# vlaxose/jstsp19

Hardware: AMD Instinct MI355X
Metric: channel-estimates/sec (batched MC) at Nt=Nr=64,K=64; NMSE vs ref (higher is better)
Workload: dtype c32 (storage and results fp32 complex; big contractions as split-f16 MFMA with fp32 accumulation, fp32-equivalent); 1 GPU; proposed_algorithm approximate Imax=100, Nt=Nr=64 Nrf=8 K=64 L=8 (N=64 M=4096 Gr=64 G2=512); Imax=100, outputs=S,Y,convergence_error, pilots=per-trial (B per trial), parallelism=trials sharded, dp1

## Files before the change

### jstsp19_amd/csrc/common.h

```cpp
#pragma once
#include <hip/hip_runtime.h>
#include <cstdint>
#include <cstdio>
#include <cstdarg>
#include <string>
#include <vector>
#include <map>
#include "../../include/jstsp.h"

namespace jstsp {

void set_error(const char *fmt, ...);

#define JSTSP_HIP(call)                                                                  \
    do {                                                                                 \
        hipError_t e_ = (call);                                                          \
        if (e_ != hipSuccess) {                                                          \
            jstsp::set_error("%s failed: %s (%s:%d)", #call, hipGetErrorString(e_),      \
                             __FILE__, __LINE__);                                        \
            return (int)e_;                                                              \
        }                                                                                \
    } while (0)

#define JSTSP_TRY(expr)                                                                  \
// ... 146 lines not shown
    bool profiling = false;
    std::map<std::string, jstsp::ProfileSlot> prof;
    std::vector<hipEvent_t> event_pool;
    int num_cus = 256;
    void *pinned = nullptr;
    size_t pinned_cap = 0, pinned_off = 0;
    hipEvent_t pinned_done = nullptr;
    bool pinned_pending = false;
    uint32_t *diag = nullptr;
    unsigned *lz_mismatch = nullptr;
    void *hpin = nullptr;
    size_t hpin_cap = 0;
    hipEvent_t hpin_done = nullptr;
    bool hpin_pending = false;
    int dict_block_hint = 0;
    int last_dict_block = 0;
    int fused_fallbacks = 0;
    float2 *unit = nullptr;
    double2 *unit64 = nullptr;
    jstsp_ctx *helper = nullptr;
    hipStream_t side[2] = {nullptr, nullptr};
    hipStream_t cu_stream[4] = {nullptr, nullptr, nullptr, nullptr};
    int cu_state = 0;
    hipStream_t bj_stream[3] = {nullptr, nullptr, nullptr};
    hipEvent_t bj_ev[6] = {nullptr, nullptr, nullptr, nullptr, nullptr, nullptr};
    hipEvent_t ev[10] = {nullptr, nullptr, nullptr, nullptr, nullptr, nullptr, nullptr, nullptr, nullptr, nullptr};
};

namespace jstsp {

struct GemmDesc {
    const float2 *A; long long sAt, sAi, sAk; int conjA;
    const float2 *B; long long sBt, sBk, sBj; int conjB;
    const float2 *B2;
    float2 *C; long long sCt; int ldc;
    const float2 *D; long long sDt; int ldd;
    float alpha, beta;
    int m, n, k, batch;
    int splitk; long long sCsplit;
    int epi;
    const TrialParams *prm;
    float2 *e_rw0, *e_w1, *e_w2, *e_w3;
    const float2 *e_r0, *e_r1, *e_r2, *e_r3;
    const float *e_f0;
    int epi_store_c;
    uint32_t *amax_x, *amax_v1, *amax_z;
// ... 3 lines not shown
    int herm_upper;
    int sa_mode;
    const float *sa_lr, *sa_lt;
    float sa_rho, sa_thr;
};
__device__ __forceinline__ float sadmm_den(float lr, float lt, float rho) { return fmaf(lr, lt, -rho); }
__device__ __forceinline__ float sadmm_dual1(float z, float r, float s, float rho) { return fmaf(rho, r - s, z); }
__device__ __forceinline__ float sadmm_soft1(float r, float z, float ir, float thr)
{
    const float v = fmaf(ir, z, r);
    const float m = fmaxf(fabsf(v) - thr, 0.f);
    return (v > 0.f) ? m : ((v < 0.f) ? -m : 0.f);
}
__device__ __forceinline__ float sadmm_rhs1(float z, float s, float a, float rho) { return fmaf(-rho, s, z) + a; }
enum { EPI_NONE = 0, EPI_UPDATE_C = 1, EPI_UPDATE_X = 2, EPI_SADMM = 3 };
enum { GEMM_MISC = 0, GEMM_CORRELATE = 1, GEMM_SYNTH = 2, GEMM_GRAM = 3 };
int launch_cgemm(jstsp_ctx *ctx, const GemmDesc &d, int tag = GEMM_MISC);

struct HPack {
    uint4 *data = nullptr;
    uint32_t *bmax = nullptr;
    int KS = 0, JT = 0, count = 0;
    long long st = 0;
};
struct HGemmDesc {
    const float2 *A; long long sAt, sAk;
    const uint32_t *amax;
    const uint4 *Bp; long long sPt;
    const uint32_t *bmax; int sbmax;
    int KS, JT;
    float2 *C; long long sCt; int ldc;
    int m, n, k, batch;
    int epi;
    const TrialParams *prm;
    const float2 *e_r0;
    float2 *e_rw0;
    uint32_t *amax_v2;
    const uint4 *Ap; long long sApt; int aKS;
    int herm_upper;
    int map_tb, map_tt;
};
int hermitian_fill_lower(jstsp_ctx *ctx, float2 *G, long long sGt, int n, int count);
int launch_hgram(jstsp_ctx *ctx, const float2 *Z, long long sZt, int rows, int cols, int count, int nsplit,
                 const uint32_t *amax, float2 *Gpart, const float2 *Z2 = nullptr,
                 const TrialParams *zprm = nullptr,
                 bool norm_only = false);
int launch_hgram3(jstsp_ctx *ctx, const float2 *X, const float2 *V1, long long sZt, int rows, int cols, int count, int nsplit,
                  const uint32_t *xmax, const uint32_t *vmax, const uint32_t *zmax, const TrialParams *prm, float2 *Gz,
                  float2 *Gx, float2 *Gv);
size_t hgemm_pack_bytes(int Kd, int J, int count);
bool hgemm_pair_shape(int m, int n, int batch);
int hgemm_absmax(jstsp_ctx *ctx, const float2 *X, long long n, long long sXt, int count, uint32_t *amax);
int hgemm_pack(jstsp_ctx *ctx, HPack &p, Arena &ar, const float2 *B, long long sBt, long long sBk, long long sBj,
               int conj, int Kd, int J, int count, long long n_contig, const uint32_t *bmax_known = nullptr);
int hgemm_repack(jstsp_ctx *ctx, const HPack &p, const float2 *B, long long sBt, long long sBk, long long sBj, int conj,
                 int Kd, int J, const uint32_t *bmax);
int launch_hgemm(jstsp_ctx *ctx, const HGemmDesc &d, const char *prof_name = nullptr);
bool use_hgemm(long long m, long long n, long long k);

enum { EIG_SVT_Q = 0, EIG_LMAX = 1, EIG_VECS = 2 };
int launch_eig(jstsp_ctx *ctx, int mode, int n, int batch, const float2 *Gpart, long long sGt,
               int nsplit, long long sGs, const TrialParams *prm, const float *tau,
               float2 *Q, float *lam_out, float2 *Vg);
bool eig_needs_global_v(int n);
int launch_eig_large(jstsp_ctx *ctx, int mode, int n, int batch, const float2 *Gpart, long long sGt, int nsplit,
                     long long sGs, const TrialParams *prm, const float *tau, float2 *Q, float *lam_out);
int launch_eig_fast(jstsp_ctx *ctx, int mode, int n, int batch, const float2 *Gpart, long long sGt, int nsplit,
                    long long sGs, const TrialParams *prm, const float *tau, float2 *Q, float *lam_out,
                    float2 *Uwarm, int warm);
int launch_eig128(jstsp_ctx *ctx, int n, int batch, const float2 *Gpart, long long sGt, int nsplit, long long sGs,
                  const TrialParams *prm, const float *tau, float2 *Q, float2 *Uwarm = nullptr, int warm = 0,
                  int max_sweeps = 16, float stop_level = 0.f);
int eig_fast_ne(int n);
struct LanczosWarm {
    float2 *x = nullptr;
    int *state = nullptr;
    unsigned *mismatch = nullptr;
// ... 32 lines not shown
```

### jstsp19_amd/csrc/hgemm.hip

```cpp
#include "solver_common.h"
#include <type_traits>

namespace jstsp {

typedef _Float16 half8 __attribute__((ext_vector_type(8)));
typedef float f32x16 __attribute__((ext_vector_type(16)));
typedef unsigned int u32x4 __attribute__((ext_vector_type(4)));

namespace {

constexpr int HBK = 32;
constexpr int FLUSH = 8;
constexpr float LO_SCALE = 1.f, LO_INV = 1.f;

__device__ __host__ inline int scale_exp(uint32_t amax_bits)
{
    const int be = (int)((amax_bits >> 23) & 0xff);
    if (be == 0 || be == 255) return 0;
    return 13 - (be - 127);
}

__device__ __forceinline__ void split2(float x, _Float16 &h, _Float16 &l)
{
    h = (_Float16)x;
// ... 6 lines not shown
    const float *p = X + (long long)t * sXt;
    float m = 0.f;
    const bool vec = ((sXt & 3) == 0) && ((n2 & 3) == 0) && (((uintptr_t)X & 15) == 0);
    if (vec) {
        const float4 *p4 = reinterpret_cast<const float4 *>(p);
        for (long long i = (long long)blockIdx.x * 256 + threadIdx.x; i < n2 / 4; i += (long long)gridDim.x * 256) {
            const float4 v = p4[i];
            m = fmaxf(fmaxf(m, fmaxf(fabsf(v.x), fabsf(v.y))), fmaxf(fabsf(v.z), fabsf(v.w)));
        }
    } else {
        for (long long i = (long long)blockIdx.x * 256 + threadIdx.x; i < n2; i += (long long)gridDim.x * 256)
            m = fmaxf(m, fabsf(p[i]));
    }
    for (int o = 32; o > 0; o >>= 1) m = fmaxf(m, __shfl_xor(m, o));
    __shared__ float sm[4];
    if ((threadIdx.x & 63) == 0) sm[threadIdx.x >> 6] = m;
    __syncthreads();
    if (threadIdx.x == 0)
        atomicMax(&amax[t], __float_as_uint(fmaxf(fmaxf(sm[0], sm[1]), fmaxf(sm[2], sm[3]))));
}

__global__ __launch_bounds__(256) void pack_b_kernel(const float2 *B, long long sBt, long long sBk, long long sBj,
                                                     int conj, int Kd, int J, int KS, int JT, const uint32_t *bmax,
                                                     uint4 *out)
{
    const int t = blockIdx.y;
    const long long idx = (long long)blockIdx.x * 256 + threadIdx.x;
    if (idx >= (long long)JT * KS * 64) return;
    const int lane = (int)(idx & 63);
    const long long blk = idx >> 6;
    const int ks = (int)(blk % KS), jt = (int)(blk / KS);
    const int j = jt * 32 + (lane & 31), k0 = ks * 16 + 8 * (lane >> 5);
    const float s = ldexpf(1.f, scale_exp(bmax[t]));
    const float sg = conj ? -s : s;
    half8 rh, rl, ih, il;
#pragma unroll
    for (int v = 0; v < 8; ++v) {
        float2 x = make_float2(0.f, 0.f);
        if (j < J && k0 + v < Kd) x = B[(long long)t * sBt + (long long)(k0 + v) * sBk + (long long)j * sBj];
        _Float16 h, l;
        split2(x.x * s, h, l); rh[v] = h; rl[v] = l;
        split2(x.y * sg, h, l); ih[v] = h; il[v] = l;
    }
    uint4 *o = out + (((long long)t * JT + jt) * KS + ks) * 256 + lane;
    o[0] = *reinterpret_cast<uint4 *>(&rh);
    o[64] = *reinterpret_cast<uint4 *>(&rl);
    o[128] = *reinterpret_cast<uint4 *>(&ih);
    o[192] = *reinterpret_cast<uint4 *>(&il);
}

__device__ __forceinline__ half8 as_half8(uint4 u) { return *reinterpret_cast<half8 *>(&u); }
__device__ __forceinline__ half8 neg_half8(uint4 u)
{
    u.x ^= 0x80008000u; u.y ^= 0x80008000u; u.z ^= 0x80008000u; u.w ^= 0x80008000u;
    return *reinterpret_cast<half8 *>(&u);
}

__device__ __forceinline__ bool block_to_trial_tile(const HGemmDesc &d, int tiles, int &t, int &tile)
{
    const int bid = blockIdx.x;
    const int xcd = bid & 7, slot = bid >> 3;
    if (d.map_tb == 0) {
        t = (slot / tiles) * 8 + xcd;
        tile = slot % tiles;
        return t < d.batch;
    }
    const int per = d.map_tb * d.map_tt;
    const int nbt = (d.batch + d.map_tb - 1) / d.map_tb;
    const int blk = (slot / per) * 8 + xcd, w = slot % per;
    t = (blk % nbt) * d.map_tb + w % d.map_tb;
    tile = (blk / nbt) * d.map_tt + w / d.map_tb;
    return t < d.batch && tile < tiles;
}

template <int EPI, bool APACK, int WJ, bool EVEN = false>
__global__ __launch_bounds__(128 * WJ, WJ == 2 ? 2 : 2) void hgemm_kernel(HGemmDesc d, int tiles_i, int tiles_j)
{
    constexpr int STG = 1024 + 512 * WJ;
    constexpr int NA = (WJ == 2) ? 8 : 4;
    __shared__ uint4 smem[2 * STG];

    const int tiles = tiles_i * tiles_j;
    int t, rem;
    if (!block_to_trial_tile(d, tiles, t, rem)) return;
    const int ti = rem % tiles_i, tj = rem / tiles_i;
    const int i0 = ti * 64, j0 = tj * 32 * WJ;
    if (d.herm_upper && i0 >= j0 + 32 * WJ) return;

    const int tid = threadIdx.x, lane = tid & 63, wave = tid >> 6;
    const int wi = wave & 1, wj = wave >> 1;

    const int ea = scale_exp(d.amax[t]);
    const int eb = scale_exp(d.bmax[(long long)t * d.sbmax]);
    const float sa = ldexpf(1.f, ea);

    const int ai = tid & 63, akg = tid >> 6;
    const bool arow = (i0 + ai) < d.m;
    const float2 *abase = APACK ? nullptr : d.A + (long long)t * d.sAt;
    const float2 *pa = APACK ? nullptr : abase + (arow ? (i0 + ai) : 0) + (long long)(NA * akg) * d.sAk;
    const int a_slot = (WJ == 2) ? ((((ai >> 5) * 2 + (akg >> 1)) * 4) * 64) + (akg & 1) * 32 + (ai & 31)
                                 : ((((ai >> 5) * 2 + (akg >> 2)) * 4) * 64) + ((akg >> 1) & 1) * 32 + (ai & 31);
    const uint4 *pb = d.Bp + (long long)t * d.sPt + ((long long)(tj * WJ) * d.KS) * 256 + lane;
    const int nst = d.KS / 2;
    const int kfull = d.k / HBK;

    struct StgF { float2 a[NA]; uint4 b0, b1, b2, b3; };
    struct StgP { u32x4 a0, a1, a2, a3; uint4 b0, b1, b2, b3; };
    using Stg = typename std::conditional<APACK, StgP, StgF>::type;
    const uint4 *pbw = pb + ((long long)(wave >> 1) * d.KS + (wave & 1)) * 256;
    const uint4 *paw = APACK ? d.Ap + (long long)t * d.sApt + lane +
                                   ((long long)(ti * 2 + (wave >> 1)) * d.KS + (wave & 1)) * 256
                             : nullptr;
    const float sa_m = arow ? sa : 0.f;
    auto load = [&](int s_in, Stg &R) {
        const int s = EVEN ? (s_in < nst ? s_in : 0) : s_in;
        const uint4 *g = pbw + (long long)(2 * s) * 256;
        const u32x4 *gn = reinterpret_cast<const u32x4 *>(g);
        const u32x4 x0 = __builtin_nontemporal_load(gn), x1 = __builtin_nontemporal_load(gn + 64),
                    x2 = __builtin_nontemporal_load(gn + 128), x3 = __builtin_nontemporal_load(gn + 192);
        R.b0 = make_uint4(x0.x, x0.y, x0.z, x0.w); R.b1 = make_uint4(x1.x, x1.y, x1.z, x1.w);
        R.b2 = make_uint4(x2.x, x2.y, x2.z, x2.w); R.b3 = make_uint4(x3.x, x3.y, x3.z, x3.w);
        if constexpr (APACK) {
            const u32x4 *ga = reinterpret_cast<const u32x4 *>(paw + (long long)(2 * s) * 256);
            R.a0 = ga[0]; R.a1 = ga[64]; R.a2 = ga[128]; R.a3 = ga[192];
        } else {
            if (EVEN || s < kfull) {
#pragma unroll
                for (int v = 0; v < NA; ++v) R.a[v] = pa[(long long)(s * HBK + v) * d.sAk];
            } else {
                const int kbase = s * HBK + NA * akg;
#pragma unroll
                for (int v = 0; v < NA; ++v) {
                    const bool ok = kbase + v < d.k;
                    const float2 *p = ok ? pa + (long long)(s * HBK + v) * d.sAk : abase;
                    const float2 x = *p;
                    R.a[v] = ok ? x : make_float2(0.f, 0.f);
                }
            }
        }
    };
    auto store = [&](const Stg &R, uint4 *buf) {
        uint4 *o = buf + 1024 + wave * 256 + lane;
        o[0] = R.b0; o[64] = R.b1; o[128] = R.b2; o[192] = R.b3;
        if constexpr (APACK) {
            u32x4 *q = reinterpret_cast<u32x4 *>(buf + wave * 256 + lane);
            q[0] = R.a0; q[64] = R.a1; q[128] = R.a2; q[192] = R.a3;
        } else {
            half8 rh = {0}, rl = {0}, ih = {0}, il = {0};
#pragma unroll
            for (int v = 0; v < NA; ++v) {
                _Float16 h, l;
                split2(R.a[v].x * sa_m, h, l); rh[v] = h; rl[v] = l;
                split2(R.a[v].y * sa_m, h, l); ih[v] = h; il[v] = l;
            }
            if constexpr (WJ == 2) {
                uint4 *q = buf + a_slot;
                q[0] = *reinterpret_cast<uint4 *>(&rh);
                q[64] = *reinterpret_cast<uint4 *>(&rl);
                q[128] = *reinterpret_cast<uint4 *>(&ih);
                q[192] = *reinterpret_cast<uint4 *>(&il);
            } else {
                uint2 *q = reinterpret_cast<uint2 *>(buf + a_slot) + (akg & 1);
                q[0] = *reinterpret_cast<uint2 *>(&rh);
                q[2 * 64] = *reinterpret_cast<uint2 *>(&rl);
                q[2 * 128] = *reinterpret_cast<uint2 *>(&ih);
                q[2 * 192] = *reinterpret_cast<uint2 *>(&il);
            }
        }
    };

    f32x16 re_h = {0}, re_l = {0}, im_h = {0}, im_l = {0};
    f32x16 Lre = {0}, Lim = {0};
    auto fold = [&]() {
#pragma unroll
        for (int r = 0; r < 16; ++r) {
            Lre[r] += re_h[r] + re_l[r] * LO_INV;
            Lim[r] += im_h[r] + im_l[r] * LO_INV;
            re_h[r] = 0.f; re_l[r] = 0.f; im_h[r] = 0.f; im_l[r] = 0.f;
        }
    };
    auto compute = [&](const uint4 *buf) {
#pragma unroll
        for (int ks = 0; ks < 2; ++ks) {
            const uint4 *fa = buf + ((wi * 2 + ks) * 4) * 64 + lane;
            const uint4 *fb = buf + 1024 + ((wj * 2 + ks) * 4) * 64 + lane;
            const uint4 uar_h = fa[0], uar_l = fa[64], uai_h = fa[128], uai_l = fa[192];
            const half8 br_h = as_half8(fb[0]), br_l = as_half8(fb[64]), bi_h = as_half8(fb[128]), bi_l = as_half8(fb[192]);
            const half8 ar_h = as_half8(uar_h), ar_l = as_half8(uar_l), ai_h = as_half8(uai_h), ai_l = as_half8(uai_l);
            const half8 nai_h = neg_half8(uai_h), nai_l = neg_half8(uai_l);
            re_h = __builtin_amdgcn_mfma_f32_32x32x16_f16(br_h, ar_h, re_h, 0, 0, 0);
            re_l = __builtin_amdgcn_mfma_f32_32x32x16_f16(br_l, ar_h, re_l, 0, 0, 0);
            im_h = __builtin_amdgcn_mfma_f32_32x32x16_f16(bi_h, ar_h, im_h, 0, 0, 0);
            im_l = __builtin_amdgcn_mfma_f32_32x32x16_f16(bi_l, ar_h, im_l, 0, 0, 0);
            re_h = __builtin_amdgcn_mfma_f32_32x32x16_f16(bi_h, nai_h, re_h, 0, 0, 0);
            re_l = __builtin_amdgcn_mfma_f32_32x32x16_f16(br_h, ar_l, re_l, 0, 0, 0);
            im_h = __builtin_amdgcn_mfma_f32_32x32x16_f16(br_h, ai_h, im_h, 0, 0, 0);
            im_l = __builtin_amdgcn_mfma_f32_32x32x16_f16(bi_h, ar_l, im_l, 0, 0, 0);
            re_l = __builtin_amdgcn_mfma_f32_32x32x16_f16(bi_l, nai_h, re_l, 0, 0, 0);
            im_l = __builtin_amdgcn_mfma_f32_32x32x16_f16(br_l, ai_h, im_l, 0, 0, 0);
            re_l = __builtin_amdgcn_mfma_f32_32x32x16_f16(bi_h, nai_l, re_l, 0, 0, 0);
            im_l = __builtin_amdgcn_mfma_f32_32x32x16_f16(br_h, ai_l, im_l, 0, 0, 0);
        }
    };
    auto stage = [&](int s, const uint4 *cur, uint4 *nxt, Stg &Rnear, Stg &Rfar) {
        if (EVEN || s + 2 < nst) load(s + 2, Rfar);
        compute(cur);
        asm volatile("" ::: "memory");
        __builtin_amdgcn_sched_barrier(0);
        if (EVEN || s + 1 < nst) store(Rnear, nxt);
        if (((s + 1) % FLUSH) == 0) fold();
        __syncthreads();
    };

    Stg R0, R1;
    uint4 *buf0 = smem, *buf1 = smem + STG;
    load(0, R0);
    if (EVEN || nst > 1) load(1, R1);
    store(R0, buf0);
    __syncthreads();

    for (int s = 0; s < nst; s += 2) {
        stage(s, buf0, buf1, R1, R0);
        if (EVEN || s + 1 < nst) stage(s + 1, buf1, buf0, R0, R1);
    }
    fold();

    const float alpha = ldexpf(1.f, -(ea + eb));
    const int gi = i0 + wi * 32 + (lane & 31);
    float2 *Cp = d.C + (long long)t * d.sCt;
    float vmax = 0.f;
    if (gi < d.m) {
#pragma unroll
        for (int r = 0; r < 16; ++r) {
            const int gj = j0 + wj * 32 + (r & 3) + 8 * (r >> 2) + 4 * (lane >> 5);
            if (gj >= d.n) continue;
            const float2 o = make_float2(Lre[r] * alpha, Lim[r] * alpha);
            const long long ix = (long long)t * d.sCt + gi + (long long)gj * d.ldc;
            if (EPI == EPI_UPDATE_C) {
                const TrialParams prm = d.prm[t];
                const float2 x = d.e_r0[ix];
                float2 v2 = d.e_rw0[ix];
                v2.x = admm_v2(prm, v2.x, x.x, o.x);
                v2.y = admm_v2(prm, v2.y, x.y, o.y);
                d.e_rw0[ix] = v2;
                vmax = fmaxf(vmax, fmaxf(fabsf(v2.x), fabsf(v2.y)));
            }
            Cp[gi + (long long)gj * d.ldc] = o;
// ... 786 lines not shown
    JSTSP_HIP(hipGetLastError());
    return 0;
}

int hgemm_pack(jstsp_ctx *ctx, HPack &p, Arena &ar, const float2 *B, long long sBt, long long sBk, long long sBj,
               int conj, int Kd, int J, int count, long long n_contig, const uint32_t *bmax_known)
{
    p.KS = 4 * ((Kd + 63) / 64);
    p.JT = 4 * ((J + 127) / 128);
    p.count = count;
    p.st = (long long)p.JT * p.KS * 256;
    p.data = ar.get<uint4>((size_t)count * p.st);
    p.bmax = ar.get<uint32_t>(count);
    JSTSP_REQUIRE(p.data && p.bmax, JSTSP_E_NOMEM, "workspace exhausted (packed dictionary)");
    if (bmax_known) JSTSP_HIP(hipMemcpyAsync(p.bmax, bmax_known, (size_t)count * sizeof(uint32_t), hipMemcpyDeviceToDevice, ctx->stream));
    else JSTSP_TRY(hgemm_absmax(ctx, B, n_contig, sBt, count, p.bmax));
    const long long slots = (long long)p.JT * p.KS * 64;
    pack_b_kernel<<<dim3((unsigned)((slots + 255) / 256), count), 256, 0, ctx->stream>>>(B, sBt, sBk, sBj, conj, Kd, J,
                                                                                         p.KS, p.JT, p.bmax, p.data);
    JSTSP_HIP(hipGetLastError());
    return 0;
}

int hgemm_repack(jstsp_ctx *ctx, const HPack &p, const float2 *B, long long sBt, long long sBk, long long sBj, int conj,
                 int Kd, int J, const uint32_t *bmax)
{
    const long long slots = (long long)p.JT * p.KS * 64;
    pack_b_kernel<<<dim3((unsigned)((slots + 255) / 256), p.count), 256, 0, ctx->stream>>>(B, sBt, sBk, sBj, conj, Kd, J,
                                                                                           p.KS, p.JT, bmax, p.data);
    JSTSP_HIP(hipGetLastError());
    return 0;
}

int launch_hgram(jstsp_ctx *ctx, const float2 *Z, long long sZt, int rows, int cols, int count, int nsplit,
                 const uint32_t *amax, float2 *Gpart, const float2 *Z2, const TrialParams *zprm, bool norm_only)
{
    JSTSP_REQUIRE(rows > 0 && rows <= 64 && cols > 0 && count > 0 && nsplit > 0, JSTSP_E_SHAPE, "hgram: bad shape");
    const long long grid = (long long)count * nsplit;
    JSTSP_REQUIRE(grid < (1ll << 31), JSTSP_E_UNSUPPORTED, "hgram grid too large");
    prof_begin(ctx, "gram");
    JSTSP_REQUIRE(!Z2 || zprm, JSTSP_E_NULL, "hgram: Z2 without per-problem scalars");
    if (norm_only && !Z2 && cols >= GRAM_HONLY_MIN_COLS) {
        if (cols % (nsplit * 2 * HBK) == 0)
            hgram_kernel<true, true><<<(unsigned)grid, 256, 0, ctx->stream>>>(Z, sZt, rows, cols, nsplit, amax, Gpart, count, Z2, zprm);
        else
            hgram_kernel<false, true><<<(unsigned)grid, 256, 0, ctx->stream>>>(Z, sZt, rows, cols, nsplit, amax, Gpart, count, Z2, zprm);
// ... 63 lines not shown
        d.map_tt = conc / d.map_tb < 1 ? 1 : conc / d.map_tb;
        if (d.map_tt > tiles) d.map_tt = (int)tiles;
        const long long nb = (long long)((d.batch + d.map_tb - 1) / d.map_tb) * ((tiles + d.map_tt - 1) / d.map_tt);
        return ((nb + 7) / 8) * 8 * d.map_tb * d.map_tt;
    }
    return (long long)((d.batch + 7) / 8) * 8 * tiles;
}

bool hgemm_pair_shape(int m, int n, int batch)
{
    return m == 64 && batch >= 2 && (long long)((batch + 1) / 2) * ((n + 127) / 128) >= 256;
}

int launch_hgemm(jstsp_ctx *ctx, const HGemmDesc &d_in, const char *prof_name)
{
    HGemmDesc d = d_in;
    JSTSP_REQUIRE(d.m > 0 && d.n > 0 && d.k > 0 && d.batch > 0, JSTSP_E_SHAPE, "hgemm: bad shape");
    JSTSP_REQUIRE(d.KS >= 2 * ((d.k + 31) / 32) && d.JT >= 2 * ((d.n + 63) / 64), JSTSP_E_ARG,
                  "hgemm: packed operand smaller than the product");
    const bool wide = !d.Ap && d.epi == EPI_NONE && d.n >= 128 && d.JT * 32 >= ((d.n + 127) / 128) * 128;
    const int tiles_i = (d.m + 63) / 64, tiles_j = wide ? (d.n + 127) / 128 : (d.n + 63) / 64;
    const bool wide_even = wide && (d.k % 32) == 0 && ((d.KS / 2) % 2) == 0 && d.KS == 2 * (d.k / 32);
    JSTSP_REQUIRE((long long)((d.batch + 7) / 8) * 8 * tiles_i * tiles_j < (1ll << 30), JSTSP_E_UNSUPPORTED, "hgemm grid too large");
    if (d.Ap && d.aKS == d.KS && d.sPt == 0 && d.sbmax == 0 && !d.herm_upper && (d.KS % 4) == 0 &&
        hgemm_pair_shape(d.m, d.n, d.batch) && d.JT * 32 >= ((d.n + 127) / 128) * 128) {
        const int npairs = (d.batch + 1) / 2, tj3 = (d.n + 127) / 128;
        d.map_tb = npairs < 4 ? npairs : 4;
        d.map_tt = 32 / d.map_tb < tj3 ? 32 / d.map_tb : tj3;
        const long long nb = (long long)((npairs + d.map_tb - 1) / d.map_tb) * ((tj3 + d.map_tt - 1) / d.map_tt);
        const long long grid3 = ((nb + 7) / 8) * 8 * d.map_tb * d.map_tt;
        JSTSP_REQUIRE(grid3 < (1ll << 31), JSTSP_E_UNSUPPORTED, "hgemm grid too large");
        if (prof_name) prof_begin(ctx, prof_name);
        constexpr int PAIR_LDS = 3 * 2048 * (int)sizeof(uint4);
        auto go = [&](auto kern, int lds) -> int {
            JSTSP_HIP(hipFuncSetAttribute(reinterpret_cast<const void *>(kern), hipFuncAttributeMaxDynamicSharedMemorySize, lds));
            hipLaunchKernelGGL(kern, dim3((unsigned)grid3), dim3(256), lds, ctx->stream, d, tj3, npairs);
            return 0;
        };
        if (d.epi == EPI_UPDATE_C) JSTSP_TRY(go(hgemm_pair_kernel<EPI_UPDATE_C, false>, PAIR_LDS));
        else if (d.k > 1024) JSTSP_TRY(go(hgemm_pair_kernel<EPI_NONE, true>, PAIR_LDS + 65536));
        else JSTSP_TRY(go(hgemm_pair_kernel<EPI_NONE, false>, PAIR_LDS));
        if (prof_name) prof_end(ctx, prof_name);
        JSTSP_HIP(hipGetLastError());
        return 0;
    }
    const int v2_mask = 1;
    const bool pack_ok = d.JT * 32 >= ((d.n + 127) / 128) * 128;
    if (d.m <= 64 && pack_ok && d.Ap && (v2_mask & 1) && d.aKS == d.KS && (d.KS % 4) == 0) {
        const int tj2 = (d.n + 127) / 128;
        const long long grid2 = hgemm_grid(d, tj2, 64);
        if (prof_name) prof_begin(ctx, prof_name);
        if (d.epi == EPI_UPDATE_C)
            hgemm2_kernel<EPI_UPDATE_C, true, 4, 2><<<(unsigned)grid2, 256, 0, ctx->stream>>>(d, tj2);
        else
            hgemm2_kernel<EPI_NONE, true, 4, 2><<<(unsigned)grid2, 256, 0, ctx->stream>>>(d, tj2);
        if (prof_name) prof_end(ctx, prof_name);
        JSTSP_HIP(hipGetLastError());
        return 0;
    }
    if (d.m <= 64 && pack_ok && !d.Ap && (v2_mask & 2) && (d.KS % 4) == 0 && d.epi == EPI_NONE && d.k <= 1024) {
        const int tj2 = (d.n + 127) / 128;
        const long long grid2 = hgemm_grid(d, tj2, 64);
        if (prof_name) prof_begin(ctx, prof_name);
        hgemm2_kernel<EPI_NONE, false, 4, 2><<<(unsigned)grid2, 256, 0, ctx->stream>>>(d, tj2);
        if (prof_name) prof_end(ctx, prof_name);
        JSTSP_HIP(hipGetLastError());
        return 0;
    }
    const long long grid = hgemm_grid(d, (long long)tiles_i * tiles_j, wide ? 32 : 64);
    if (prof_name) prof_begin(ctx, prof_name);
    if (wide_even) {
        hgemm_kernel<EPI_NONE, false, 4, true><<<(unsigned)grid, 512, 0, ctx->stream>>>(d, tiles_i, tiles_j);
    } else if (wide) {
        hgemm_kernel<EPI_NONE, false, 4><<<(unsigned)grid, 512, 0, ctx->stream>>>(d, tiles_i, tiles_j);
    } else if (d.Ap) {
        JSTSP_REQUIRE(d.aKS == d.KS, JSTSP_E_ARG, "hgemm: packed a and b operands disagree on the k padding");
        if (d.epi == EPI_UPDATE_C)
            hgemm_kernel<EPI_UPDATE_C, true, 2><<<(unsigned)grid, 256, 0, ctx->stream>>>(d, tiles_i, tiles_j);
        else
            hgemm_kernel<EPI_NONE, true, 2><<<(unsigned)grid, 256, 0, ctx->stream>>>(d, tiles_i, tiles_j);
    } else if (d.epi == EPI_UPDATE_C)
        hgemm_kernel<EPI_UPDATE_C, false, 2><<<(unsigned)grid, 256, 0, ctx->stream>>>(d, tiles_i, tiles_j);
    else
        hgemm_kernel<EPI_NONE, false, 2><<<(unsigned)grid, 256, 0, ctx->stream>>>(d, tiles_i, tiles_j);
    if (prof_name) prof_end(ctx, prof_name);
    JSTSP_HIP(hipGetLastError());
    return 0;
}

}
```

### jstsp19_amd/csrc/proposed.hip

```cpp
#include "solver_common.h"
#include <cstdio>
#include <cmath>
#include <cstdlib>
#include <algorithm>

namespace jstsp {

struct ProposedWS {
    float2 *X, *V1, *V2, *C, *Xs, *Y, *ZK, *Zb, *Zb2;
    float *invD;
    float2 *V, *RV, *Res, *RRes, *S, *P1;
    float2 *Tc, *W;
    float2 *GA, *GB;
    TrialParams *prm;
    int32_t *rank;
    double *ce;
    float *lam;
    GramWS gz, gn;
    bool h2 = false;
    HPack Bc, Bs;
    uint32_t *kmax = nullptr, *wmax = nullptr;
    uint32_t *nmax = nullptr, *zmax = nullptr;
    bool h2g = false;
    HPack GBp;
    HPack Wp;
    HPack Kp;
    uint32_t *pmax = nullptr;
};

static int gram3_nsplit(int N, int M, int G2, bool want_ce)
{
    const int chunk = 1024;
    if (!(want_ce && N <= 64 && N <= M && use_hgemm(N, G2, M))) return 0;
    return std::max(1, std::min(32, (M + chunk - 1) / chunk));
}

static size_t proposed_bytes(int N, int M, int Gr, int G2, int batch, int nA, int nB, bool angles,
                             bool want_ce, int Imax)
{
    const size_t nm = (size_t)N * M, g = (size_t)Gr * G2, ng = (size_t)N * G2;
    size_t b = 0;
    b += rnd256(3 * batch * nm * sizeof(float2)) + 6 * rnd256(batch * nm * sizeof(float2));
    b += rnd256(batch * nm * sizeof(float));
    b += 6 * rnd256(batch * g * sizeof(float2));
    b += 2 * rnd256(batch * ng * sizeof(float2));
    b += rnd256((size_t)nA * Gr * Gr * sizeof(float2)) + rnd256((size_t)nB * G2 * G2 * sizeof(float2));
    b += rnd256(batch * sizeof(TrialParams));
    if (angles) b += rnd256(batch * g * sizeof(int32_t));
    b += rnd256((size_t)batch * 3 * Imax * sizeof(double));
    b += rnd256(3 * (size_t)batch * sizeof(float));
    const int ns3 = gram3_nsplit(N, M, G2, want_ce);
    b += GramWS::bytes(N, M, batch, true, ns3);
    if (want_ce) b += GramWS::bytes(N, M, 3 * batch, false, ns3);
    if (use_hgemm(N, G2, M))
        b += hgemm_pack_bytes(M, G2, nB) + hgemm_pack_bytes(G2, M, nB) + 2 * rnd256(8 * batch * sizeof(uint32_t)) +
             hgemm_pack_bytes(G2, N, batch);
    if (use_hgemm(N, G2, M) && nB == 1 && hgemm_pair_shape(N, G2, batch))
        b += rnd256((size_t)batch * 2 * (4 * ((M + 63) / 64)) * 256 * sizeof(uint4));
    if (use_hgemm(Gr, G2, G2)) b += hgemm_pack_bytes(G2, G2, nB) + rnd256(2 * batch * sizeof(uint32_t));
    return b;
}

static int proposed_alloc(Arena &a, ProposedWS &w, int N, int M, int Gr, int G2, int batch, int nA, int nB,
                          bool angles, bool want_ce, int Imax)
{
    const size_t nm = (size_t)N * M, g = (size_t)Gr * G2, ng = (size_t)N * G2;
    w.X = a.get<float2>(3 * batch * nm);
    w.V1 = w.X ? w.X + batch * nm : nullptr;
    w.V2 = w.X ? w.X + 2 * batch * nm : nullptr;
    w.C = a.get<float2>(batch * nm); w.Xs = a.get<float2>(batch * nm); w.Y = a.get<float2>(batch * nm);
    w.ZK = a.get<float2>(batch * nm);
    w.Zb = a.get<float2>(batch * nm);
    w.Zb2 = a.get<float2>(batch * nm);
    w.invD = a.get<float>(batch * nm);
    w.V = a.get<float2>(batch * g); w.RV = a.get<float2>(batch * g); w.Res = a.get<float2>(batch * g);
    w.RRes = a.get<float2>(batch * g); w.S = a.get<float2>(batch * g); w.P1 = a.get<float2>(batch * g);
    w.Tc = a.get<float2>(batch * ng); w.W = a.get<float2>(batch * ng);
    w.GA = a.get<float2>((size_t)nA * Gr * Gr); w.GB = a.get<float2>((size_t)nB * G2 * G2);
    w.prm = a.get<TrialParams>(batch);
    w.rank = angles ? a.get<int32_t>(batch * g) : nullptr;
    w.ce = a.get<double>((size_t)batch * 3 * Imax);
    w.lam = a.get<float>(3 * (size_t)batch);
// ... 149 lines not shown
    const Mat Am{A, strideA, N}, Bm{B, strideB, G2};
    const int toep_env = tn.toeplitz;
    int toep_gt = 0;
    bool toep_probed = false;
    const Mat GAm{w.GA, strideA ? (long long)Gr * Gr : 0, Gr}, GBm{w.GB, strideB ? (long long)G2 * G2 : 0, G2};
    float2 *GAlo = nullptr;
    if (approx) {
        GAlo = ctx->arena.get<float2>((size_t)nA * Gr * Gr);
        JSTSP_REQUIRE(GAlo, JSTSP_E_NOMEM, "proposed_algorithm: workspace exhausted (Gram refinement)");
        JSTSP_TRY(gram_f64(ctx, 'L', A, strideA, N, Gr, nA, w.GA, (long long)Gr * Gr, GAlo));
    } else
    JSTSP_TRY(gemm(ctx, 'C', 'N', Gr, Gr, N, nA, Am, Am, w.GA, (long long)Gr * Gr, Gr));
    if (toep_env != 0 && known_gt && strideB) {
        toep_gt = known_gt;
        toep_probed = true;
    } else
    if (toep_env != 0 && (long long)G2 * M < (1ll << 31) && approx) {
        JSTSP_TRY(fused_probe_toeplitz(ctx, ctx->arena, B, strideB, G2, M, nB, &toep_gt));
        toep_probed = true;
    }
    if (w.h2) {
        JSTSP_TRY(hgemm_pack(ctx, w.Bc, ctx->arena, B, strideB, G2, 1, 1, M, G2, nB, (long long)G2 * M));
    }
    if (approx) {
        if (toep_gt && toep_env >= 2 && M >= G2 / toep_gt) {
            float2 *G0 = ctx->arena.get<float2>((size_t)nB * toep_gt * G2), *G0lo = ctx->arena.get<float2>((size_t)nB * toep_gt * G2);
            JSTSP_REQUIRE(G0 && G0lo, JSTSP_E_NOMEM, "workspace exhausted (G_B block row)");
            GemmDesc dg = make_gemm('N', 'C', toep_gt, G2, M, nB, Bm, Bm, G0, (long long)toep_gt * G2, toep_gt);
            dg.force_m64 = 1; dg.C_lo = G0lo;
            JSTSP_TRY(launch_cgemm(ctx, dg, GEMM_MISC));
            JSTSP_TRY(toeplitz_gram_assemble(ctx, B, strideB, G2, M, toep_gt, nB, G0, G0lo, w.GB, nullptr));
            ctx->last_dict_block = toep_gt;
        } else {
            GemmDesc dg = make_gemm('N', 'C', G2, G2, M, nB, Bm, Bm, w.GB, (long long)G2 * G2, G2);
            dg.force_m64 = 1; dg.herm_upper = 1;
            JSTSP_TRY(launch_cgemm(ctx, dg, GEMM_MISC));
            JSTSP_TRY(hermitian_fill_lower(ctx, w.GB, (long long)G2 * G2, G2, nB));
        }
    } else if (w.h2) {
        {
            HGemmDesc hb{B, strideB, G2, w.Bc.bmax, w.Bc.data, w.Bc.st, w.Bc.bmax, 1, w.Bc.KS, w.Bc.JT, w.GB,
                         (long long)G2 * G2, G2, G2, G2, M, nB, EPI_NONE, nullptr, nullptr, nullptr};
            hb.herm_upper = 1;
            JSTSP_TRY(launch_hgemm(ctx, hb, nullptr));
            JSTSP_TRY(hermitian_fill_lower(ctx, w.GB, (long long)G2 * G2, G2, nB));
        }
    } else
    JSTSP_TRY(gemm(ctx, 'N', 'C', G2, G2, M, nB, Bm, Bm, w.GB, (long long)G2 * G2, G2));

    if (w.h2g && approx)
        JSTSP_TRY(hgemm_pack(ctx, w.GBp, ctx->arena, w.GB, strideB ? (long long)G2 * G2 : 0, 1, G2, 0, G2, G2, nB,
                             (long long)G2 * G2));
    float2 *PA = nullptr, *PB = nullptr;
    if (!approx) {
        JSTSP_TRY(diag_reset(ctx));
        if (pinv_fits(N, Gr)) {
            PA = ctx->arena.get<float2>((size_t)nA * Gr * N);
            JSTSP_REQUIRE(PA, JSTSP_E_NOMEM, "proposed_algorithm 'std': workspace exhausted");
            JSTSP_TRY(launch_pinv(ctx, N, Gr, nA, A, strideA, N, PA, (long long)Gr * N, Gr));
        }
        if (pinv_fits(G2, M)) {
            PB = ctx->arena.get<float2>((size_t)nB * M * G2);
            JSTSP_REQUIRE(PB, JSTSP_E_NOMEM, "proposed_algorithm 'std': workspace exhausted");
            JSTSP_TRY(launch_pinv(ctx, G2, M, nB, B, strideB, G2, PB, (long long)M * G2, M));
        }
        float2 *GAi = PA ? nullptr : ctx->arena.get<float2>((size_t)nA * Gr * Gr);
        float2 *GBi = PB ? nullptr : ctx->arena.get<float2>((size_t)nB * G2 * G2);
        JSTSP_REQUIRE((PA || GAi) && (PB || GBi), JSTSP_E_NOMEM, "proposed_algorithm 'std': workspace exhausted");
        const size_t mark = ctx->arena.off;
        if (!PA) {
            JSTSP_TRY(hermitian_inverse(ctx, Gr, nA, w.GA, GAi));
            ctx->arena.off = mark;
            JSTSP_HIP(hipMemcpyAsync(w.GA, GAi, (size_t)nA * Gr * Gr * sizeof(float2), hipMemcpyDeviceToDevice, st));
        }
        if (!PB) {
// ... 112 lines not shown
        } else if (w.h2) {
            if (!fz) JSTSP_TRY(hgemm_absmax(ctx, w.ZK, snm, snm, batch, w.kmax));
            HGemmDesc hc{w.ZK, snm, N, w.kmax, w.Bc.data, strideB ? w.Bc.st : 0, w.Bc.bmax, strideB ? 1 : 0, w.Bc.KS,
                         w.Bc.JT, w.Tc, sng, N, N, G2, M, batch, EPI_NONE, nullptr, nullptr, nullptr};
            if (w.Kp.data && !strideB && w.Kp.KS == w.Bc.KS) {
                w.Kp.bmax = w.kmax;
                JSTSP_TRY(hgemm_repack(ctx, w.Kp, w.ZK, snm, N, 1, 0, M, N, w.kmax));
                hc.Ap = w.Kp.data; hc.sApt = w.Kp.st; hc.aKS = w.Kp.KS;
            }
            JSTSP_TRY(launch_hgemm(ctx, hc, "correlate"));
        } else
        JSTSP_TRY(gemm(ctx, 'N', 'C', N, G2, M, batch, Mat{w.ZK, snm, N}, Bm, w.Tc, sng, N, 1.f, nullptr, 0, 0,
                       0.f, GEMM_CORRELATE));
        const long long cnt_ll = std::min<long long>(10 + 5ll * (it + 1), (long long)g);
        const Mat GAl{GAlo, strideA ? (long long)Gr * Gr : 0, Gr};
        auto second_factor = [&](float2 *out, uint32_t *pm, bool exact) -> int {
            if (exact || !w.h2g) {
                GemmDesc dr = make_gemm('N', 'N', Gr, G2, G2, batch, Mat{w.P1, sg, Gr}, GBm, out, sg, Gr);
                dr.force_m64 = exact ? 1 : 0;
                return launch_cgemm(ctx, dr, GEMM_MISC);
            }
            HGemmDesc hg{w.P1, sg, Gr, pm, w.GBp.data, strideB ? w.GBp.st : 0, w.GBp.bmax, strideB ? 1 : 0,
                         w.GBp.KS, w.GBp.JT, out, sg, Gr, Gr, G2, G2, batch, EPI_NONE, nullptr, nullptr, nullptr};
            return launch_hgemm(ctx, hg, nullptr);
        };
        auto apply_R = [&](const float2 *Xin, float2 *out, bool exact) -> int {
            uint32_t *pm = w.pmax ? w.pmax + (size_t)(apply_no++ & 1) * batch : nullptr;
            if (exact && rv_fused1) {
                JSTSP_TRY(launch_grad_refresh_p1(ctx, Xin, w.GA, GAlo, strideA ? (long long)Gr * Gr : 0, w.P1, G2, batch));
                return second_factor(out, pm, exact);
            }
            if (exact) JSTSP_TRY(gemm(ctx, 'N', 'N', Gr, G2, Gr, batch, GAl, Mat{Xin, sg, Gr}, w.P1, sg, Gr));
            GemmDesc dp = make_gemm('N', 'N', Gr, G2, Gr, batch, GAm, Mat{Xin, sg, Gr}, w.P1, sg, Gr, 1.f, exact ? w.P1 : nullptr, sg,
                                    Gr, exact ? 1.f : 0.f);
            dp.amax_out = w.h2g ? pm : nullptr;
            JSTSP_TRY(launch_cgemm(ctx, dp, GEMM_MISC));
            return second_factor(out, pm, exact);
        };
        if (approx) {
            const bool refreshed = refresh_at(it);
            if (refreshed && rv_early) {
                JSTSP_HIP(hipStreamWaitEvent(sm, ev_rv, 0));
                rv_early = false;
            } else if (refreshed) JSTSP_TRY(apply_R(w.V, w.RV, true));
            if (svt_split && tn.grad_fused != 0 && w.h2g && grad_fused_shape(N, Gr, G2)) {
                uint32_t *pm = w.pmax + (size_t)(apply_no++ & 1) * batch;
// ... 334 lines not shown
```

Baseline: 845.1 channel-estimates/s.

## Pack Hermitian Gram operand as triangular image and mirror tiles via transposed LDS reads

The packed f16 image of the Hermitian dictionary Gram matrix GB now stores only the upper block-triangle. The 64x128 hgemm instance reads the missing lower tiles from their mirrored upper tiles, using a lane swizzle on the LDS store, ds_read_tr16 transposed reads and a sign flip on the imaginary part for conjugation. This roughly halves the packed operand footprint and the global traffic of the repeated second-factor product, at the cost of more address arithmetic and a more complex, fragile kernel path. The pair-kernel dynamic-LDS attribute call is also cached per context, with a fallback to the generic path if it fails.

```diff
diff --git a/jstsp19_amd/csrc/common.h b/jstsp19_amd/csrc/common.h
--- a/jstsp19_amd/csrc/common.h
+++ b/jstsp19_amd/csrc/common.h
@@ -192,6 +192,7 @@
     hipStream_t side[2] = {nullptr, nullptr};
     hipStream_t cu_stream[4] = {nullptr, nullptr, nullptr, nullptr};
     int cu_state = 0;
+    int pair_lds_ok[3] = {0, 0, 0};
     hipStream_t bj_stream[3] = {nullptr, nullptr, nullptr};
     hipEvent_t bj_ev[6] = {nullptr, nullptr, nullptr, nullptr, nullptr, nullptr};
     hipEvent_t ev[10] = {nullptr, nullptr, nullptr, nullptr, nullptr, nullptr, nullptr, nullptr, nullptr, nullptr};
@@ -241,7 +242,13 @@
     uint32_t *bmax = nullptr;
     int KS = 0, JT = 0, count = 0;
     long long st = 0;
-};
+    int hs = 0;
+};
+inline __host__ __device__ int herm_tile_off(int jt, int hs)
+{
+    const int jb = jt >> hs;
+    return (2 << hs) * (jb + 1) * ((jb << hs) / 2 + (jt & ((1 << hs) - 1)));
+}
 struct HGemmDesc {
     const float2 *A; long long sAt, sAk;
     const uint32_t *amax;
@@ -258,6 +265,7 @@
     const uint4 *Ap; long long sApt; int aKS;
     int herm_upper;
     int map_tb, map_tt;
+    int herm_hs;
 };
 int hermitian_fill_lower(jstsp_ctx *ctx, float2 *G, long long sGt, int n, int count);
 int launch_hgram(jstsp_ctx *ctx, const float2 *Z, long long sZt, int rows, int cols, int count, int nsplit,
@@ -272,6 +280,8 @@
 int hgemm_absmax(jstsp_ctx *ctx, const float2 *X, long long n, long long sXt, int count, uint32_t *amax);
 int hgemm_pack(jstsp_ctx *ctx, HPack &p, Arena &ar, const float2 *B, long long sBt, long long sBk, long long sBj,
                int conj, int Kd, int J, int count, long long n_contig, const uint32_t *bmax_known = nullptr);
+size_t hgemm_pack_herm_bytes(int G2, int hs, int count);
+int hgemm_pack_herm(jstsp_ctx *ctx, HPack &p, Arena &ar, const float2 *G, long long sGt, int G2, int hs, int count);
 int hgemm_repack(jstsp_ctx *ctx, const HPack &p, const float2 *B, long long sBt, long long sBk, long long sBj, int conj,
                  int Kd, int J, const uint32_t *bmax);
 int launch_hgemm(jstsp_ctx *ctx, const HGemmDesc &d, const char *prof_name = nullptr);
diff --git a/jstsp19_amd/csrc/hgemm.hip b/jstsp19_amd/csrc/hgemm.hip
--- a/jstsp19_amd/csrc/hgemm.hip
+++ b/jstsp19_amd/csrc/hgemm.hip
@@ -52,7 +52,7 @@
 
 __global__ __launch_bounds__(256) void pack_b_kernel(const float2 *B, long long sBt, long long sBk, long long sBj,
                                                      int conj, int Kd, int J, int KS, int JT, const uint32_t *bmax,
-                                                     uint4 *out)
+                                                     uint4 *out, int hs = 0, long long st = 0)
 {
     const int t = blockIdx.y;
     const long long idx = (long long)blockIdx.x * 256 + threadIdx.x;
@@ -60,6 +60,7 @@
     const int lane = (int)(idx & 63);
     const long long blk = idx >> 6;
     const int ks = (int)(blk % KS), jt = (int)(blk / KS);
+    if (hs && ks >= (2 << hs) * ((jt >> hs) + 1)) return;
     const int j = jt * 32 + (lane & 31), k0 = ks * 16 + 8 * (lane >> 5);
     const float s = ldexpf(1.f, scale_exp(bmax[t]));
     const float sg = conj ? -s : s;
@@ -72,7 +73,8 @@
         split2(x.x * s, h, l); rh[v] = h; rl[v] = l;
         split2(x.y * sg, h, l); ih[v] = h; il[v] = l;
     }
-    uint4 *o = out + (((long long)t * JT + jt) * KS + ks) * 256 + lane;
+    uint4 *o = hs ? out + (long long)t * st + (long long)(herm_tile_off(jt, hs) + ks) * 256 + lane
+                  : out + (((long long)t * JT + jt) * KS + ks) * 256 + lane;
     o[0] = *reinterpret_cast<uint4 *>(&rh);
     o[64] = *reinterpret_cast<uint4 *>(&rl);
     o[128] = *reinterpret_cast<uint4 *>(&ih);
@@ -103,9 +105,10 @@
     return t < d.batch && tile < tiles;
 }
 
-template <int EPI, bool APACK, int WJ, bool EVEN = false>
+template <int EPI, bool APACK, int WJ, bool EVEN = false, bool HERM = false>
 __global__ __launch_bounds__(128 * WJ, WJ == 2 ? 2 : 2) void hgemm_kernel(HGemmDesc d, int tiles_i, int tiles_j)
 {
+    static_assert(!HERM || (WJ == 4 && EVEN && !APACK && EPI == EPI_NONE), "the Hermitian image is read by the 64 x 128 instance");
     constexpr int STG = 1024 + 512 * WJ;
     constexpr int NA = (WJ == 2) ? 8 : 4;
     __shared__ uint4 smem[2 * STG];
@@ -138,6 +141,11 @@
     struct StgP { u32x4 a0, a1, a2, a3; uint4 b0, b1, b2, b3; };
     using Stg = typename std::conditional<APACK, StgP, StgF>::type;
     const uint4 *pbw = pb + ((long long)(wave >> 1) * d.KS + (wave & 1)) * 256;
+    const int hs = HERM ? d.herm_hs : 0;
+    const int wvu = HERM ? __builtin_amdgcn_readfirstlane(wave) : 0;
+    const int hjt = HERM ? min(tj * WJ + (wvu >> 1), (d.n >> 5) - 1) : 0, hjb = hjt >> hs;
+    const uint4 *pbh = HERM ? d.Bp + (long long)t * d.sPt + lane + (long long)(wvu & 1) * 256 : nullptr;
+    const int hown = HERM ? herm_tile_off(hjt, hs) : 0;
     const uint4 *paw = APACK ? d.Ap + (long long)t * d.sApt + lane +
                                    ((long long)(ti * 2 + (wave >> 1)) * d.KS + (wave & 1)) * 256
                              : nullptr;
@@ -145,6 +153,8 @@
     auto load = [&](int s_in, Stg &R) {
         const int s = EVEN ? (s_in < nst ? s_in : 0) : s_in;
         const uint4 *g = pbw + (long long)(2 * s) * 256;
+        if constexpr (HERM)
+            g = pbh + (long long)(((s >> hs) > hjb) ? herm_tile_off(s, hs) + 2 * hjt : hown + 2 * s) * 256;
         const u32x4 *gn = reinterpret_cast<const u32x4 *>(g);
         const u32x4 x0 = __builtin_nontemporal_load(gn), x1 = __builtin_nontemporal_load(gn + 64),
                     x2 = __builtin_nontemporal_load(gn + 128), x3 = __builtin_nontemporal_load(gn + 192);
@@ -169,8 +179,9 @@
             }
         }
     };
-    auto store = [&](const Stg &R, uint4 *buf) {
-        uint4 *o = buf + 1024 + wave * 256 + lane;
+    auto store = [&](const Stg &R, uint4 *buf, int s) {
+        const int blane = (HERM && (s >> hs) > hjb) ? lane ^ (4 * ((lane >> 5) + 2 * (wvu & 1))) : lane;
+        uint4 *o = buf + 1024 + wave * 256 + blane;
         o[0] = R.b0; o[64] = R.b1; o[128] = R.b2; o[192] = R.b3;
         if constexpr (APACK) {
             u32x4 *q = reinterpret_cast<u32x4 *>(buf + wave * 256 + lane);
@@ -209,13 +220,37 @@
             re_h[r] = 0.f; re_l[r] = 0.f; im_h[r] = 0.f; im_l[r] = 0.f;
         }
     };
-    auto compute = [&](const uint4 *buf) {
+    typedef short s16x4 __attribute__((ext_vector_type(4)));
+    typedef __attribute__((address_space(3))) s16x4 lds_s16x4;
+    typedef unsigned int u32x2 __attribute__((ext_vector_type(2)));
+    auto *lbase = (__attribute__((address_space(3))) unsigned char *)smem;
+    const int trc = ((lane >> 1) & 1) + 2 * ((lane >> 4) & 1);
+    const uint32_t troff = HERM ? (uint32_t)((1024 + ((wj * 2 + ((lane >> 4) & 1)) * 4) * 64) * 16 + ((lane >> 1) & 1) * 512 +
+                                             ((8 * (lane >> 5) + ((lane >> 2) & 3)) ^ (4 * trc)) * 16 + (lane & 1) * 8)
+                                : 0u;
+    auto compute = [&](const uint4 *buf, auto mir_c) {
+        constexpr bool mir = decltype(mir_c)::value;
 #pragma unroll
         for (int ks = 0; ks < 2; ++ks) {
             const uint4 *fa = buf + ((wi * 2 + ks) * 4) * 64 + lane;
             const uint4 *fb = buf + 1024 + ((wj * 2 + ks) * 4) * 64 + lane;
             const uint4 uar_h = fa[0], uar_l = fa[64], uai_h = fa[128], uai_l = fa[192];
-            const half8 br_h = as_half8(fb[0]), br_l = as_half8(fb[64]), bi_h = as_half8(fb[128]), bi_l = as_half8(fb[192]);
+            half8 br_h, br_l, bi_h, bi_l;
+            if constexpr (HERM && mir) {
+                const uint32_t o = (uint32_t)(buf - smem) * 16 + troff + ks * 256, o1 = o ^ 64u;
+                u32x4 f[4];
+#pragma unroll
+                for (int p = 0; p < 4; ++p) {
+                    const u32x2 lo = __builtin_bit_cast(u32x2, __builtin_amdgcn_ds_read_tr16_b64_v4i16((lds_s16x4 *)(lbase + o + p * 1024)));
+                    const u32x2 hi = __builtin_bit_cast(u32x2, __builtin_amdgcn_ds_read_tr16_b64_v4i16((lds_s16x4 *)(lbase + o1 + p * 1024)));
+                    f[p] = u32x4{lo.x, lo.y, hi.x, hi.y};
+                }
+                f[2] ^= 0x80008000u; f[3] ^= 0x80008000u;
+                br_h = *reinterpret_cast<half8 *>(&f[0]); br_l = *reinterpret_cast<half8 *>(&f[1]);
+                bi_h = *reinterpret_cast<half8 *>(&f[2]); bi_l = *reinterpret_cast<half8 *>(&f[3]);
+            } else {
+                br_h = as_half8(fb[0]); br_l = as_half8(fb[64]); bi_h = as_half8(fb[128]); bi_l = as_half8(fb[192]);
+            }
             const half8 ar_h = as_half8(uar_h), ar_l = as_half8(uar_l), ai_h = as_half8(uai_h), ai_l = as_half8(uai_l);
             const half8 nai_h = neg_half8(uai_h), nai_l = neg_half8(uai_l);
             re_h = __builtin_amdgcn_mfma_f32_32x32x16_f16(br_h, ar_h, re_h, 0, 0, 0);
@@ -232,12 +267,12 @@
             im_l = __builtin_amdgcn_mfma_f32_32x32x16_f16(br_h, ai_l, im_l, 0, 0, 0);
         }
     };
-    auto stage = [&](int s, const uint4 *cur, uint4 *nxt, Stg &Rnear, Stg &Rfar) {
+    auto stage = [&](int s, const uint4 *cur, uint4 *nxt, Stg &Rnear, Stg &Rfar, auto mir_c) {
         if (EVEN || s + 2 < nst) load(s + 2, Rfar);
-        compute(cur);
+        compute(cur, mir_c);
         asm volatile("" ::: "memory");
         __builtin_amdgcn_sched_barrier(0);
-        if (EVEN || s + 1 < nst) store(Rnear, nxt);
+        if (EVEN || s + 1 < nst) store(Rnear, nxt, s + 1);
         if (((s + 1) % FLUSH) == 0) fold();
         __syncthreads();
     };
@@ -246,13 +281,19 @@
     uint4 *buf0 = smem, *buf1 = smem + STG;
     load(0, R0);
     if (EVEN || nst > 1) load(1, R1);
-    store(R0, buf0);
+    store(R0, buf0, 0);
     __syncthreads();
 
-    for (int s = 0; s < nst; s += 2) {
-        stage(s, buf0, buf1, R1, R0);
-        if (EVEN || s + 1 < nst) stage(s + 1, buf1, buf0, R0, R1);
-    }
+    const int nsd = HERM ? min(nst, (hjb + 1) << hs) : nst;
+    for (int s = 0; s < nsd; s += 2) {
+        stage(s, buf0, buf1, R1, R0, std::false_type{});
+        if (EVEN || s + 1 < nst) stage(s + 1, buf1, buf0, R0, R1, std::false_type{});
+    }
+    if constexpr (HERM)
+        for (int s = nsd; s < nst; s += 2) {
+            stage(s, buf0, buf1, R1, R0, std::true_type{});
+            stage(s + 1, buf1, buf0, R0, R1, std::true_type{});
+        }
     fold();
 
     const float alpha = ldexpf(1.f, -(ea + eb));
@@ -1085,6 +1126,33 @@
     return 0;
 }
 
+size_t hgemm_pack_herm_bytes(int G2, int hs, int count)
+{
+    const size_t nb = (size_t)G2 / (32u << hs);
+    return rnd256((size_t)count * ((size_t)1 << (2 * hs)) * nb * (nb + 1) * 4096) + rnd256((size_t)count * sizeof(uint32_t));
+}
+
+int hgemm_pack_herm(jstsp_ctx *ctx, HPack &p, Arena &ar, const float2 *G, long long sGt, int G2, int hs, int count)
+{
+    JSTSP_REQUIRE(hs >= 1 && hs <= 3 && G2 > 0 && G2 % (32 << hs) == 0, JSTSP_E_ARG, "hgemm: bad Hermitian image");
+    const int nb = G2 / (32 << hs);
+    p.KS = G2 / 16;
+    p.JT = 4 * ((G2 + 127) / 128);
+    p.count = count;
+    p.hs = hs;
+    p.st = (long long)herm_tile_off(nb << hs, hs) * 256;
+    p.data = ar.get<uint4>((size_t)count * p.st);
+    p.bmax = ar.get<uint32_t>(count);
+    JSTSP_REQUIRE(p.data && p.bmax, JSTSP_E_NOMEM, "workspace exhausted (packed Hermitian operand)");
+    JSTSP_TRY(hgemm_absmax(ctx, G, (long long)G2 * G2, sGt, count, p.bmax));
+    const int jt = G2 / 32;
+    const long long slots = (long long)jt * p.KS * 64;
+    pack_b_kernel<<<dim3((unsigned)((slots + 255) / 256), count), 256, 0, ctx->stream>>>(G, sGt, 1, G2, 0, G2, G2, p.KS, jt, p.bmax,
+                                                                                         p.data, hs, p.st);
+    JSTSP_HIP(hipGetLastError());
+    return 0;
+}
+
 int hgemm_repack(jstsp_ctx *ctx, const HPack &p, const float2 *B, long long sBt, long long sBk, long long sBj, int conj,
                  int Kd, int J, const uint32_t *bmax)
 {
@@ -1194,6 +1262,9 @@
     const int tiles_i = (d.m + 63) / 64, tiles_j = wide ? (d.n + 127) / 128 : (d.n + 63) / 64;
     const bool wide_even = wide && (d.k % 32) == 0 && ((d.KS / 2) % 2) == 0 && d.KS == 2 * (d.k / 32);
     JSTSP_REQUIRE((long long)((d.batch + 7) / 8) * 8 * tiles_i * tiles_j < (1ll << 30), JSTSP_E_UNSUPPORTED, "hgemm grid too large");
+    JSTSP_REQUIRE(!d.herm_hs || (wide_even && d.n == d.k && d.herm_hs >= 1 && d.herm_hs <= 3 && d.n % (32 << d.herm_hs) == 0 &&
+                                 !d.herm_upper && (d.sPt == 0 || d.sPt == (long long)herm_tile_off(d.n >> 5, d.herm_hs) * 256)),
+                  JSTSP_E_ARG, "hgemm: this product cannot take a Hermitian image");
     if (d.Ap && d.aKS == d.KS && d.sPt == 0 && d.sbmax == 0 && !d.herm_upper && (d.KS % 4) == 0 &&
         hgemm_pair_shape(d.m, d.n, d.batch) && d.JT * 32 >= ((d.n + 127) / 128) * 128) {
         const int npairs = (d.batch + 1) / 2, tj3 = (d.n + 127) / 128;
@@ -1202,19 +1273,28 @@
         const long long nb = (long long)((npairs + d.map_tb - 1) / d.map_tb) * ((tj3 + d.map_tt - 1) / d.map_tt);
         const long long grid3 = ((nb + 7) / 8) * 8 * d.map_tb * d.map_tt;
         JSTSP_REQUIRE(grid3 < (1ll << 31), JSTSP_E_UNSUPPORTED, "hgemm grid too large");
-        if (prof_name) prof_begin(ctx, prof_name);
         constexpr int PAIR_LDS = 3 * 2048 * (int)sizeof(uint4);
-        auto go = [&](auto kern, int lds) -> int {
-            JSTSP_HIP(hipFuncSetAttribute(reinterpret_cast<const void *>(kern), hipFuncAttributeMaxDynamicSharedMemorySize, lds));
+        auto go = [&](auto kern, int lds, int slot) -> bool {
+            if (ctx->pair_lds_ok[slot] == 0) {
+                const hipError_t e = hipFuncSetAttribute(reinterpret_cast<const void *>(kern), hipFuncAttributeMaxDynamicSharedMemorySize, lds);
+                if (e != hipSuccess) (void)hipGetLastError();
+                ctx->pair_lds_ok[slot] = e == hipSuccess ? 1 : -1;
+            }
+            if (ctx->pair_lds_ok[slot] < 0) return false;
+            if (prof_name) prof_begin(ctx, prof_name);
             hipLaunchKernelGGL(kern, dim3((unsigned)grid3), dim3(256), lds, ctx->stream, d, tj3, npairs);
+            if (prof_name) prof_end(ctx, prof_name);
+            return true;
+        };
+        bool done;
+        if (d.epi == EPI_UPDATE_C) done = go(hgemm_pair_kernel<EPI_UPDATE_C, false>, PAIR_LDS, 0);
+        else if (d.k > 1024) done = go(hgemm_pair_kernel<EPI_NONE, true>, PAIR_LDS + 65536, 1);
+        else done = go(hgemm_pair_kernel<EPI_NONE, false>, PAIR_LDS, 2);
+        if (done) {
+            JSTSP_HIP(hipGetLastError());
             return 0;
-        };
-        if (d.epi == EPI_UPDATE_C) JSTSP_TRY(go(hgemm_pair_kernel<EPI_UPDATE_C, false>, PAIR_LDS));
-        else if (d.k > 1024) JSTSP_TRY(go(hgemm_pair_kernel<EPI_NONE, true>, PAIR_LDS + 65536));
-        else JSTSP_TRY(go(hgemm_pair_kernel<EPI_NONE, false>, PAIR_LDS));
-        if (prof_name) prof_end(ctx, prof_name);
-        JSTSP_HIP(hipGetLastError());
-        return 0;
+        }
+        d.map_tb = d.map_tt = 0;
     }
     const int v2_mask = 1;
     const bool pack_ok = d.JT * 32 >= ((d.n + 127) / 128) * 128;
@@ -1241,7 +1321,9 @@
     }
     const long long grid = hgemm_grid(d, (long long)tiles_i * tiles_j, wide ? 32 : 64);
     if (prof_name) prof_begin(ctx, prof_name);
-    if (wide_even) {
+    if (d.herm_hs) {
+        hgemm_kernel<EPI_NONE, false, 4, true, true><<<(unsigned)grid, 512, 0, ctx->stream>>>(d, tiles_i, tiles_j);
+    } else if (wide_even) {
         hgemm_kernel<EPI_NONE, false, 4, true><<<(unsigned)grid, 512, 0, ctx->stream>>>(d, tiles_i, tiles_j);
     } else if (wide) {
         hgemm_kernel<EPI_NONE, false, 4><<<(unsigned)grid, 512, 0, ctx->stream>>>(d, tiles_i, tiles_j);
diff --git a/jstsp19_amd/csrc/proposed.hip b/jstsp19_amd/csrc/proposed.hip
--- a/jstsp19_amd/csrc/proposed.hip
+++ b/jstsp19_amd/csrc/proposed.hip
@@ -35,6 +35,24 @@
     return std::max(1, std::min(32, (M + chunk - 1) / chunk));
 }
 
+static int gb_image_hs(int G2, int gt)
+{
+    if (tune().fused == 2 || G2 < 128 || G2 % 64 != 0) return 0;
+    int hs = 1;
+    while ((32 << hs) < gt) ++hs;
+    return (hs <= 3 && G2 % (32 << hs) == 0) ? hs : 0;
+}
+
+static size_t gb_image_bytes(int G2, int nB)
+{
+    if (!gb_image_hs(G2, 0)) return hgemm_pack_bytes(G2, G2, nB);
+    size_t b = hgemm_pack_herm_bytes(G2, 1, nB);
+    if (tune().toeplitz >= 2)
+        for (int gt = 128; gt <= 256 && 2 * gt <= G2; gt *= 2)
+            if (G2 % gt == 0) b = std::max(b, hgemm_pack_herm_bytes(G2, gb_image_hs(G2, gt), nB));
+    return b;
+}
+
 static size_t proposed_bytes(int N, int M, int Gr, int G2, int batch, int nA, int nB, bool angles,
                              bool want_ce, int Imax)
 {
@@ -57,7 +75,7 @@
              hgemm_pack_bytes(G2, N, batch);
     if (use_hgemm(N, G2, M) && nB == 1 && hgemm_pair_shape(N, G2, batch))
         b += rnd256((size_t)batch * 2 * (4 * ((M + 63) / 64)) * 256 * sizeof(uint4));
-    if (use_hgemm(Gr, G2, G2)) b += hgemm_pack_bytes(G2, G2, nB) + rnd256(2 * batch * sizeof(uint32_t));
+    if (use_hgemm(Gr, G2, G2)) b += gb_image_bytes(G2, nB) + rnd256(2 * batch * sizeof(uint32_t));
     return b;
 }
 
@@ -253,6 +271,7 @@
     if (w.h2) {
         JSTSP_TRY(hgemm_pack(ctx, w.Bc, ctx->arena, B, strideB, G2, 1, 1, M, G2, nB, (long long)G2 * M));
     }
+    int gb_gt = 0;
     if (approx) {
         if (toep_gt && toep_env >= 2 && M >= G2 / toep_gt) {
             float2 *G0 = ctx->arena.get<float2>((size_t)nB * toep_gt * G2), *G0lo = ctx->arena.get<float2>((size_t)nB * toep_gt * G2);
@@ -261,6 +280,7 @@
             dg.force_m64 = 1; dg.C_lo = G0lo;
             JSTSP_TRY(launch_cgemm(ctx, dg, GEMM_MISC));
             JSTSP_TRY(toeplitz_gram_assemble(ctx, B, strideB, G2, M, toep_gt, nB, G0, G0lo, w.GB, nullptr));
+            gb_gt = toep_gt;
             ctx->last_dict_block = toep_gt;
         } else {
             GemmDesc dg = make_gemm('N', 'C', G2, G2, M, nB, Bm, Bm, w.GB, (long long)G2 * G2, G2);
@@ -279,9 +299,13 @@
     } else
     JSTSP_TRY(gemm(ctx, 'N', 'C', G2, G2, M, nB, Bm, Bm, w.GB, (long long)G2 * G2, G2));
 
-    if (w.h2g && approx)
-        JSTSP_TRY(hgemm_pack(ctx, w.GBp, ctx->arena, w.GB, strideB ? (long long)G2 * G2 : 0, 1, G2, 0, G2, G2, nB,
-                             (long long)G2 * G2));
+    if (w.h2g && approx) {
+        if (const int hs = gb_image_hs(G2, gb_gt))
+            JSTSP_TRY(hgemm_pack_herm(ctx, w.GBp, ctx->arena, w.GB, strideB ? (long long)G2 * G2 : 0, G2, hs, nB));
+        else
+            JSTSP_TRY(hgemm_pack(ctx, w.GBp, ctx->arena, w.GB, strideB ? (long long)G2 * G2 : 0, 1, G2, 0, G2, G2, nB,
+                                 (long long)G2 * G2));
+    }
     float2 *PA = nullptr, *PB = nullptr;
     if (!approx) {
         JSTSP_TRY(diag_reset(ctx));
@@ -440,6 +464,7 @@
             }
             HGemmDesc hg{w.P1, sg, Gr, pm, w.GBp.data, strideB ? w.GBp.st : 0, w.GBp.bmax, strideB ? 1 : 0,
                          w.GBp.KS, w.GBp.JT, out, sg, Gr, Gr, G2, G2, batch, EPI_NONE, nullptr, nullptr, nullptr};
+            hg.herm_hs = w.GBp.hs;
             return launch_hgemm(ctx, hg, nullptr);
         };
         auto apply_R = [&](const float2 *Xin, float2 *out, bool exact) -> int {
```

After: 844.7 channel-estimates/s. About the same (-0.0%).
